# FederatedAI/FATE-LLM

Measured on AMD Instinct MI355X. Metric: GB/s param buffer reconstructed from (seed,scalar) list, device-resident, higher is better.
Workload: dtype bf16

## Files before the change

fate-llm_amd/csrc/fks_dev_update.h:

```cpp
#pragma once
#include <hip/hip_runtime.h>
#include <hip/hip_bf16.h>

#include "fks_internal.h"
#include "fks_dev_lds.h"

namespace fks {
namespace {

typedef __bf16 bf16x2_t __attribute__((ext_vector_type(2)));
__device__ __forceinline__ float rbf_cvt(float x) {
  const f32x2_t v = {0.0f, x};
  return __builtin_bit_cast(float, __builtin_convertvector(v, bf16x2_t));
}
__device__ __forceinline__ float rbf(float x) { return rbf_cvt(x); }
__device__ __forceinline__ float rhf(float x) {
  asm volatile("" : "+v"(x));
  return static_cast<float>(static_cast<_Float16>(x));
}

template <int DT>
struct Traits;

typedef __attribute__((address_space(1))) float gf32;
typedef __attribute__((address_space(1))) uint16_t gu16;
typedef __attribute__((address_space(1))) _Float16 gf16;

typedef __attribute__((address_space(1))) uint32_t gu32;

typedef __attribute__((address_space(1))) uint64_t gu64;

template <>
struct Traits<FKS_F32> {
  typedef uint64_t Pair;
  __device__ static Pair load_pair(uint64_t a) { return *reinterpret_cast<const gu64*>(a); }
  __device__ static void store_pair(uint64_t a, Pair v) { *reinterpret_cast<gu64*>(a) = v; }
  __device__ static uint32_t lo(Pair v) { return (uint32_t)v; }
  __device__ static uint32_t hi(Pair v) { return (uint32_t)(v >> 32); }
  __device__ static Pair pack(uint32_t l, uint32_t h) { return (uint64_t)l | ((uint64_t)h << 32); }
  __device__ static uint32_t bits(float v) { return __float_as_uint(v); }
  __device__ static uint32_t load_raw(uint64_t p, int64_t i) { return reinterpret_cast<const gu32*>(p)[i]; }
  __device__ static float cvt(uint32_t r) { return __uint_as_float(r); }
  __device__ static float load(uint64_t p, int64_t i) { return reinterpret_cast<const gf32*>(p)[i]; }
  __device__ static void store(uint64_t p, int64_t i, float v) { reinterpret_cast<gf32*>(p)[i] = v; }
  __device__ static float rnd(float x) { return x; }
};

template <>
struct Traits<FKS_BF16> {
  typedef uint32_t Pair;
  __device__ static Pair load_pair(uint64_t a) { return *reinterpret_cast<const gu32*>(a); }
  __device__ static void store_pair(uint64_t a, Pair v) { *reinterpret_cast<gu32*>(a) = v; }
  __device__ static uint32_t lo(Pair v) { return v & 0xffffu; }
  __device__ static uint32_t hi(Pair v) { return v >> 16; }
  __device__ static Pair pack(uint32_t l, uint32_t h) { return (l & 0xffffu) | (h << 16); }
  __device__ static uint32_t bits(float v) { return __float_as_uint(v) >> 16; }
  __device__ static uint32_t load_raw(uint64_t p, int64_t i) { return reinterpret_cast<const gu16*>(p)[i]; }
  __device__ static float cvt(uint32_t r) { return __uint_as_float(r << 16); }
  __device__ static float load(uint64_t p, int64_t i) {
    return __uint_as_float((uint32_t)reinterpret_cast<const gu16*>(p)[i] << 16);
  }
  __device__ static void store(uint64_t p, int64_t i, float v) {
    reinterpret_cast<gu16*>(p)[i] = (uint16_t)(__float_as_uint(v) >> 16);
  }
  __device__ static float rnd(float x) { return rbf(x); }
};

template <>
struct Traits<FKS_F16> {
  typedef uint32_t Pair;
  __device__ static Pair load_pair(uint64_t a) { return *reinterpret_cast<const gu32*>(a); }
  __device__ static void store_pair(uint64_t a, Pair v) { *reinterpret_cast<gu32*>(a) = v; }
  __device__ static uint32_t lo(Pair v) { return v & 0xffffu; }
  __device__ static uint32_t hi(Pair v) { return v >> 16; }
  __device__ static Pair pack(uint32_t l, uint32_t h) { return (l & 0xffffu) | (h << 16); }
  __device__ static uint32_t bits(float v) { return __builtin_bit_cast(uint16_t, static_cast<_Float16>(v)); }
  __device__ static uint32_t load_raw(uint64_t p, int64_t i) { return reinterpret_cast<const gu16*>(p)[i]; }
  __device__ static float cvt(uint32_t r) { return static_cast<float>(__builtin_bit_cast(_Float16, (uint16_t)r)); }
  __device__ static float load(uint64_t p, int64_t i) { return static_cast<float>(reinterpret_cast<const gf16*>(p)[i]); }
  __device__ static void store(uint64_t p, int64_t i, float v) { reinterpret_cast<gf16*>(p)[i] = static_cast<_Float16>(v); }
  __device__ static float rnd(float x) { return rhf(x); }
};

template <>
struct Traits<kDtF32Libm> : Traits<FKS_F32> {};
constexpr bool is_f32(int dt) { return dt == FKS_F32 || dt == kDtF32Libm; }

template <int DT>
__device__ __forceinline__ float apply_one(float p, float z, float g, float lr, float wd, bool has_wd, int mode,
                                           float ps, bool upd = true) {
  using TR = Traits<DT>;
  if (mode == kModeDelta) return __fmaf_rn(g, z, p);
  if (mode == kModePerturb || mode == kModePerturbUpdate) {
    p = TR::rnd(p + TR::rnd(ps * z));
    if (mode == kModePerturb || !upd) return p;
  }
  if (mode == kModeUpdate || mode == kModePerturbUpdate) {
    const float gz = TR::rnd(g * z);
    const float t2 = TR::rnd(gz + TR::rnd(wd * p));
    const float t = has_wd ? t2 : gz;
    return TR::rnd(p - TR::rnd(lr * t));
  }
  return z;
}

template <int DT>
__device__ __forceinline__ float dev_value_g(const float* v) {
  const float g = __int_as_float(__builtin_amdgcn_readfirstlane(__float_as_int(v[0])));
  return is_f32(DT) ? g : Traits<DT>::rnd(g);
}
__device__ __forceinline__ bool dev_value_apply(const float* v) {
  return __int_as_float(__builtin_amdgcn_readfirstlane(__float_as_int(v[1]))) != 0.0f;
}

template <int DT>
__device__ __forceinline__ f32x2_t rnd2(f32x2_t x) {
  f32x2_t r;
  r.x = Traits<DT>::rnd(x.x);
  r.y = Traits<DT>::rnd(x.y);
  return r;
}

template <int DT, int MODE>
__device__ __forceinline__ f32x2_t apply_tail(f32x2_t p, f32x2_t gz, float lr, float wd, bool has_wd) {
  f32x2_t t;
  if (MODE == kModeUpdateNoWd || MODE == kModeUpdateWdPos0) {
    t = gz;
  } else if (MODE == kModeUpdateWd0) {
    const f32x2_t ww = {wd, wd};
    t = __builtin_elementwise_fma(ww, p, gz);
  } else {
    const f32x2_t t2 = rnd2<DT>(gz + rnd2<DT>(wd * p));
    if (MODE == kModeUpdateWd) {
      t = t2;
    } else {
      t.x = has_wd ? t2.x : gz.x;
      t.y = has_wd ? t2.y : gz.y;
    }
  }
  return rnd2<DT>(p - rnd2<DT>(lr * t));
}

template <int DT, int MODE>
__device__ __forceinline__ f32x2_t apply_pair(f32x2_t p, f32x2_t z, float g, float lr, float wd, bool has_wd,
                                              float ps, bool upd = true) {
  if (MODE == kModeDelta) {
    const f32x2_t gg = {g, g};
    return __builtin_elementwise_fma(gg, z, p);
  }
  if (MODE == kModePerturb || MODE == kModePerturbUpdate) {
    p = rnd2<DT>(p + rnd2<DT>(ps * z));
    if (MODE == kModePerturb || !upd) return p;
  }
  if (MODE == kModeUpdate || MODE == kModeUpdateWd || MODE == kModeUpdateNoWd || MODE == kModePerturbUpdate ||
      MODE == kModeUpdateWd0 || MODE == kModeUpdateWdPos0)
    return apply_tail<DT, MODE>(p, rnd2<DT>(g * z), lr, wd, has_wd);
  return z;
}

__device__ __forceinline__ float mul_f16_ref(float a, float b, bool once) {
  if (once) {
    uint32_t r = 0;
    asm volatile("v_fma_mixlo_f16 %0, %1, %2, 0" : "+v"(r) : "v"(a), "v"(b));
    return (float)__builtin_bit_cast(_Float16, (uint16_t)(r & 0xffffu));
  }
  return rhf(a * b);
}
template <int MODE>
__device__ __forceinline__ f32x2_t apply_pair_f16dev(f32x2_t p, f32x2_t z, float g, float lr, float wd, bool has_wd,
                                                     float ps, bool upd, const bool (&once)[2],
                                                     const bool (&wd_once)[2]) {
  float q[2] = {p.x, p.y};
  const float zz[2] = {z.x, z.y};
  const bool use_wd = MODE == kModeUpdateNoWd ? false
                      : (MODE == kModeUpdateWd || MODE == kModeUpdateWd0 || MODE == kModeUpdateWdPos0) ? true
                                                                                                          : has_wd;
#pragma unroll
  for (int i = 0; i < 2; i++) {
    if (MODE == kModePerturb || MODE == kModePerturbUpdate) {
      q[i] = rhf(q[i] + mul_f16_ref(ps, zz[i], once[i]));
      if (MODE == kModePerturb || !upd) continue;
    }
    const float gz = mul_f16_ref(g, zz[i], once[i]);
    const float t = use_wd ? rhf(gz + mul_f16_ref(wd, q[i], wd_once[i])) : gz;
    q[i] = rhf(q[i] - mul_f16_ref(lr, t, once[i]));
  }
  return (f32x2_t){q[0], q[1]};
}

}
}
```

fate-llm_amd/csrc/fks_device.hip:

```cpp
#include <hip/hip_runtime.h>
#include <hip/hip_bf16.h>

#include <atomic>
#include <type_traits>
#include <mutex>

#include "fks_internal.h"
#include "fks_bitslice.h"
#define FKS_HD __device__ __forceinline__
#include "fks_libm.h"

constexpr int kDbMinWaves = 4;
constexpr int kZrUnroll = 2;
constexpr int kSm2MinWaves = 8;
constexpr int kBsFence = 8;
#ifndef FKS_BS_LAG
#define FKS_BS_LAG 36
#endif
#ifndef FKS_BS_R_VMEM
#define FKS_BS_R_VMEM 3
#endif
#ifndef FKS_PHX_VEC_ITEMS
#define FKS_PHX_VEC_ITEMS 8
#endif
#ifndef FKS_BS_WGTIME
#define FKS_BS_WGTIME 0
#endif

#include "fks_dev_lds.h"
#include "fks_dev_update.h"
#include "fks_dev_mt.h"
#include "fks_dev_zgen.h"
#include "fks_kern_jump.h"
#include "fks_kern_apply.h"
#include "fks_kern_slice.h"
#include "fks_kern_irregular.h"
#include "fks_kern_philox.h"
#include "fks_kern_selfcheck.h"

namespace fks {

int launch_delta_apply(const DeltaApplyDesc* d, int n, int64_t max_numel, const float* delta, void* stream) {
  const int64_t blocks = std::min<int64_t>(std::max<int64_t>(1, (max_numel + 255) / 256), 2048);
  hipLaunchKernelGGL(fks_delta_apply_kernel, dim3((unsigned)blocks, (unsigned)n), dim3(256), 0, (hipStream_t)stream,
                     d, delta);
  return (int)hipGetLastError();
}

static size_t apply_lds_bytes() { return (size_t)kLdsTabBytes + (size_t)kLdsStBytes; }

int device_cu_count() {
  int dev = 0, n = 0;
  if (hipGetDevice(&dev) != hipSuccess) return 256;
  if (hipDeviceGetAttribute(&n, hipDeviceAttributeMultiprocessorCount, dev) != hipSuccess || n <= 0) return 256;
  return n;
}

class PerDevice {
 public:
  template <class F>
  int run(F&& f) {
    int dev = 0;
    if (hipGetDevice(&dev) != hipSuccess || dev < 0 || dev >= 64) return -FKS_EINVAL;
    const uint64_t bit = 1ull << dev;
    if (done_.load(std::memory_order_acquire) & bit) return 0;
    std::lock_guard<std::mutex> lk(mu_);
    if (done_.load(std::memory_order_relaxed) & bit) return 0;
    const int e = f();
    if (e == 0) done_.fetch_or(bit, std::memory_order_release);
    return e;
  }

 private:
  std::mutex mu_;
  std::atomic<uint64_t> done_{0};
};

static int ensure_tables() {
  static PerDevice once;
  return once.run([] {
    const Tables& t = tables();
    static float buf[3 * 2048];
    for (int i = 0; i < 256; i++) {
      buf[i] = t.r_bf16[i];
      buf[256 + i] = t.c_bf16[i];
      buf[512 + i] = t.s_bf16[i];
    }
    hipError_t e = hipMemcpyToSymbol(HIP_SYMBOL(c_tab_bf16), buf, sizeof(float) * 768, 0, hipMemcpyHostToDevice);
    if (e != hipSuccess) return (int)e;
    for (int i = 0; i < 2048; i++) {
      buf[i] = t.r_f16[i];
      buf[2048 + i] = t.c_f16[i];
      buf[4096 + i] = t.s_f16[i];
    }
    e = hipMemcpyToSymbol(HIP_SYMBOL(c_tab_f16), buf, sizeof(buf), 0, hipMemcpyHostToDevice);
    return (int)e;
  });
}

template <class K>
static int ensure_lds_attr(PerDevice& once, K* fn, int bytes) {
  return once.run([&] {
    return (int)hipFuncSetAttribute(reinterpret_cast<const void*>(fn), hipFuncAttributeMaxDynamicSharedMemorySize,
                                    bytes);
  });
}

template <int... Vs>
struct IntList {};
template <int... Vs, class F>
static int dispatch(IntList<Vs...>, int v, F&& f) {
  int r = -FKS_ENOTSUP;
  (void)((v == Vs && (r = f(std::integral_constant<int, Vs>{}), true)) || ...);
  return r;
}

int launch_jump(const JumpArgs& a, int nseeds, void* stream) {
  const size_t lds = sizeof(uint32_t) * (size_t)kJumpLds2Words;
  static PerDevice attr;
  if (int e = ensure_lds_attr(attr, &fks_jump_kernel, (int)lds)) return e;
  dim3 grid((unsigned)nseeds, (unsigned)((a.nchunks + a.chunks_per_wg - 1) / a.chunks_per_wg));
  hipLaunchKernelGGL(fks_jump_kernel, grid, dim3(kJumpThreads), lds, (hipStream_t)stream, a);
  return (int)hipGetLastError();
}

template <int DT, int MODE, bool FULL, bool DB = false>
static int launch_apply_f(const ApplyArgs& a, void* stream) {
  const size_t lds = FULL ? apply_lds_bytes()
                          : (size_t)kLdsTabBytes + (size_t)((DB ? 2 : 1) * a.nseeds + 1) * kWinBytes;
  static PerDevice attr;
  if (int e = ensure_lds_attr(attr, &fks_apply_kernel<DT, MODE, FULL, DB>, (int)apply_lds_bytes())) return e;
  hipLaunchKernelGGL((fks_apply_kernel<DT, MODE, FULL, DB>), dim3((unsigned)a.nchunks),
                     dim3(DB ? kDbThreads : kApplyThreads), lds, (hipStream_t)stream, a);
  return (int)hipGetLastError();
}

template <int DT, int MODE, int ZM = 0>
static int launch_small2(const ApplyArgs& a, void* stream) {
  const size_t lds = (size_t)kLdsTabBytes + (size_t)(2 * a.nseeds + 1) * kWinBytes;
  static PerDevice attr;
  constexpr int kMaxLds = kLdsTabBytes + (2 * kSmallK + 1) * kWinBytes;
  if (int e = ensure_lds_attr(attr, &fks_small2_kernel<DT, MODE, ZM>, kMaxLds)) return e;
  hipLaunchKernelGGL((fks_small2_kernel<DT, MODE, ZM>), dim3((unsigned)a.nchunks), dim3(kSm2Threads), lds,
                     (hipStream_t)stream, a);
  return (int)hipGetLastError();
}

template <int DT, int MODE>
static int launch_apply_t(const ApplyArgs& a, void* stream) {
  if (a.nseeds == kMaxSeedsPerPass) return launch_apply_f<DT, MODE, true>(a, stream);
  if constexpr (DT == FKS_BF16) {
    if (a.zmode == 1 && a.nseeds == 1 && MODE == kModePerturb) return launch_small2<DT, MODE, 1>(a, stream);
    if (a.zmode == 2 && a.nseeds == 1 &&
        (MODE == kModePerturb || MODE == kModePerturbUpdate || MODE == kModeUpdate || MODE == kModeUpdateWd ||
         MODE == kModeUpdateNoWd || MODE == kModeUpdateWd0)) {
      hipLaunchKernelGGL((fks_zreplay_kernel<MODE>), dim3((unsigned)a.nchunks), dim3(kZrThreads), (size_t)3 * 1024,
                         (hipStream_t)stream, a);
      return (int)hipGetLastError();
    }
  }
  if (a.zmode == 2) return -FKS_ENOTSUP;
  if (a.nseeds <= kSmallK && DT != FKS_F16) return launch_small2<DT == FKS_F16 ? FKS_F32 : DT, MODE>(a, stream);
  if (a.nseeds <= kSmallK) return launch_apply_f<DT, MODE, false, true>(a, stream);
  return launch_apply_f<DT, MODE, false>(a, stream);
}

int launch_apply(int dtype, const ApplyArgs& a, void* stream) {
  if (a.nseeds < 1 || a.nseeds > kMaxSeedsPerPass || a.nchunks < 1) return -FKS_EINVAL;
  if (dtype == FKS_BF16) {
    int e = ensure_tables();
    if (e) return e;
  }
  using Modes = IntList<kModeUpdate, kModeUpdateWd, kModeUpdateNoWd, kModeUpdateWd0, kModePerturb, kModePerturbUpdate,
                        kModeWriteZ, kModeDelta>;
  return dispatch(IntList<FKS_F32, kDtF32Libm, FKS_BF16>{}, dtype, [&](auto dt) {
    return dispatch(Modes{}, a.mode,
                    [&](auto m) { return launch_apply_t<decltype(dt)::value, decltype(m)::value>(a, stream); });
  });
}

template <int MODE, bool FULL>
static int launch_apply_bs_m(const ApplyBsArgs& a, void* stream) {
  static PerDevice attr;
  if (int e = ensure_lds_attr(attr, &fks_apply_bs_kernel<MODE, FULL>, kBsLdsBytes)) return e;
  hipLaunchKernelGGL((fks_apply_bs_kernel<MODE, FULL>), dim3((unsigned)(a.split ? a.nchunks / 2 : a.nchunks)),
                     dim3(kBsThreads), kBsLdsBytes, (hipStream_t)stream, a);
  return (int)hipGetLastError();
}

template <int MODE>
static int launch_apply_bs_t(const ApplyBsArgs& a, void* stream) {
  const bool full = a.nseeds == (a.split ? kBsSeeds : kBsPassSeeds);
  return full ? launch_apply_bs_m<MODE, true>(a, stream) : launch_apply_bs_m<MODE, false>(a, stream);
}

int launch_apply_bs(const ApplyBsArgs& a, void* stream) {
  if (a.nseeds < 1 || a.nseeds > (a.split ? kBsSeeds : kBsPassSeeds) || a.nchunks < 1 ||
      (a.split && a.nchunks % 2))
    return -FKS_EINVAL;
  int e = ensure_tables();
  if (e) return e;
  return dispatch(IntList<kModeUpdate, kModeUpdateWd, kModeUpdateNoWd, kModeUpdateWd0, kModeDelta>{}, a.mode,
                  [&](auto m) { return launch_apply_bs_t<decltype(m)::value>(a, stream); });
}

template <int MODE>
static int launch_irregular_m(const IrrArgs& a, void* stream) {
  const size_t lds = (size_t)kIrrLogfOff + kLdsLogfBytes;
  static PerDevice attr;
  if (int e = ensure_lds_attr(attr, &fks_irregular_kernel<MODE>, (int)lds)) return e;
  hipLaunchKernelGGL((fks_irregular_kernel<MODE>), dim3((unsigned)a.nchunks), dim3(kApplyThreads), lds,
                     (hipStream_t)stream, a);
  return (int)hipGetLastError();
}

int launch_philox_fast_radius_check(uint32_t* counts, void* stream) {
  hipLaunchKernelGGL(fks_philox_fast_radius_kernel, dim3(kSqrtDomainBlocks), dim3(256), 0, (hipStream_t)stream, counts);
  return (int)hipGetLastError();
}

int launch_philox_radius_check(uint32_t* counts, void* stream) {
  hipLaunchKernelGGL(fks_philox_radius_kernel, dim3(kSqrtDomainBlocks), dim3(256), 0, (hipStream_t)stream, counts);
  return (int)hipGetLastError();
}

int launch_sqrt_domain_check(uint32_t* counts, void* stream) {
  hipLaunchKernelGGL(fks_sqrt_domain_kernel, dim3(kSqrtDomainBlocks), dim3(256), 0, (hipStream_t)stream, counts);
  return (int)hipGetLastError();
}

int device_max_threads_per_cu() {
  int dev = 0, n = 0;
  if (hipGetDevice(&dev) != hipSuccess) return 2048;
  if (hipDeviceGetAttribute(&n, hipDeviceAttributeMaxThreadsPerMultiProcessor, dev) != hipSuccess || n <= 0) return 2048;
  return n;
}

static int phx_vec_maxk() {
  static const int v = [] {
    const char* s = std::getenv("FKS_PHX_VEC_MAXK");
    return (s && *s) ? std::atoi(s) : kPhxSeeds;
  }();
  return v;
}

template <int MODE>
static int launch_philox_m(const PhiloxArgs& a, void* stream) {
  const int64_t items = a.item_hi - a.item_lo;
  if (items <= 0) return 0;
  if (a.nseeds <= phx_vec_maxk() && a.item_lo % kPhxVec == 0 && items % kPhxVec == 0) {
    const int64_t vitems = items / kPhxVec;
    const int64_t blocks = std::min<int64_t>((vitems + 255) / 256, (int64_t)device_cu_count() * 16);
    const size_t lds = a.nt <= kPhxLdsTensors ? sizeof(PhxTensor) * (size_t)a.nt : 0;
    hipLaunchKernelGGL((fks_philox_vec_kernel<MODE>), dim3((unsigned)blocks), dim3(256), lds, (hipStream_t)stream, a);
    return (int)hipGetLastError();
  }
  const int64_t blocks = std::min<int64_t>((items + 255) / 256, (int64_t)device_cu_count() * 16);
  hipLaunchKernelGGL((fks_philox_kernel<MODE>), dim3((unsigned)blocks), dim3(256), 0, (hipStream_t)stream, a);
  return (int)hipGetLastError();
}

int launch_philox(const PhiloxArgs& a, void* stream) {
  if (a.nseeds < 1 || a.nt < 1) return -FKS_EINVAL;
  using Modes = IntList<kModeUpdate, kModeUpdateWd, kModeUpdateNoWd, kModeUpdateWd0, kModeUpdateWdPos0, kModePerturb,
                        kModePerturbUpdate, kModeWriteZ, kModeDelta>;
  return dispatch(Modes{}, a.mode, [&](auto m) { return launch_philox_m<decltype(m)::value>(a, stream); });
}

int launch_irregular(const IrrArgs& a, void* stream) {
  if (a.nseeds < 1 || a.nseeds > kMaxSeedsPerPass) return -FKS_EINVAL;
  int e = ensure_tables();
  if (e) return e;
  return dispatch(IntList<kModeUpdate, kModePerturb, kModePerturbUpdate, kModeWriteZ, kModeDelta>{}, a.mode,
                  [&](auto m) { return launch_irregular_m<decltype(m)::value>(a, stream); });
}

}
```

fate-llm_amd/csrc/fks_kern_slice.h:

```cpp
#pragma once
#include <hip/hip_runtime.h>

#include "fks_internal.h"
#include "fks_bitslice.h"
#include "fks_dev_lds.h"
#include "fks_dev_update.h"
#include "fks_dev_zgen.h"

namespace fks {
namespace {

constexpr int kBsChunkBytes = kMtN * 16;
constexpr int kBsStateBytes = 8 * kBsChunkBytes;
constexpr int kBsTabBytes = 256 * 4 + 256 * 8;
constexpr uint32_t kBsFlagOff = kBsTabBytes + 2 * kBsStateBytes;
constexpr uint32_t kBsProgOff = kBsFlagOff + 8;
constexpr uint32_t kBsProg1Off = kBsProgOff + 4 * 6;
constexpr int kBsLdsBytes = (int)kBsProg1Off + 4 * 6;
static_assert(kBsLdsBytes <= 163840, "slice kernel LDS");
constexpr int kBsWaves = kBsHalfThreads / 64;
constexpr int kBsTaskWords = 128;

__device__ __forceinline__ void bs_store_row(uint32_t ra, const uint32_t (&x)[32]) {
#pragma unroll
  for (int q = 0; q < 8; q++) {
    const u32x4_t v = {x[4 * q], x[4 * q + 1], x[4 * q + 2], x[4 * q + 3]};
    lds_st4(ra + q * kBsChunkBytes, v);
  }
}

__device__ __forceinline__ uint32_t bs_flag_load(uint32_t off) {
  return *(volatile const lds_u32_t*)(size_t)off;
}
__device__ __forceinline__ void bs_flag_store(uint32_t off, uint32_t v) {
  asm volatile("" ::: "memory");
  __builtin_amdgcn_s_waitcnt(0xC07F);
  *(volatile lds_u32_t*)(size_t)off = v;
}

template <int S>
__device__ __forceinline__ uint32_t bs_index(uint32_t w, int c) {
  switch (c) {
    case 0: return bs::byte_x<0, S>(w);
    case 1: return bs::byte_x<1, S>(w);
    case 2: return bs::byte_x<2, S>(w);
    default: return bs::byte_x<3, S>(w);
  }
}

#if FKS_BS_WGTIME
__device__ uint64_t g_bs_wgtime[4096][16];
extern "C" int fks_debug_bs_wgtime(uint64_t* out, int nblocks) {
  return (int)hipMemcpyFromSymbol(out, HIP_SYMBOL(g_bs_wgtime), sizeof(uint64_t) * 16 * (size_t)nblocks, 0,
                                  hipMemcpyDeviceToHost);
}
#endif

template <int MODE, bool FULL>
__global__ __launch_bounds__(kBsThreads, 1) void fks_apply_bs_kernel(ApplyBsArgs a) {
  extern __shared__ __attribute__((aligned(16))) uint32_t lds32[];
  if ((uint32_t)(size_t)(lds_u32_t*)lds32 != 0u) __builtin_trap();
  const int tid = threadIdx.x;
  const int lane = tid & 63;
#if FKS_BS_WGTIME
  if (tid == 0) g_bs_wgtime[blockIdx.x][0] = __builtin_amdgcn_s_memrealtime();
  auto stamp = [&]() { if (lane == 0) g_bs_wgtime[blockIdx.x][1 + (tid >> 6)] = __builtin_amdgcn_s_memrealtime(); };
#else
  auto stamp = [&]() {};
#endif
  const int half = __builtin_amdgcn_readfirstlane(tid >= kBsHalfThreads ? 1 : 0);
  const int ht = tid - half * kBsHalfThreads;
  const int hw = __builtin_amdgcn_readfirstlane(ht >> 6);
  const bool split = a.split != 0;
  const int c = split ? 2 * (int)blockIdx.x + half : (int)blockIdx.x;
  const int nA = FULL ? kBsSeeds : split ? a.nseeds : (a.nseeds + 1) / 2;
  const int nseeds = FULL ? kBsSeeds : (half && !split ? a.nseeds - nA : nA);
  const int sfirst = half && !split ? nA : 0;
  const int64_t b0 = a.chunk_block[split ? c : 2 * c], b1 = a.chunk_block[split ? c + 1 : 2 * c + 2];
  const int nwords = (int)(kMtN * (b1 - b0));
  const int ntask = (nwords + kBsTaskWords - 1) / kBsTaskWords;
  const uint32_t sbase = kBsTabBytes + (uint32_t)half * kBsStateBytes;
  const uint32_t flag = kBsFlagOff + 4u * (uint32_t)half;

  for (int i = tid; i < 256; i += kBsThreads) {
    reinterpret_cast<float*>((uint8_t*)lds32)[i] = c_tab_bf16[i];
    reinterpret_cast<float2*>((uint8_t*)lds32 + 1024)[i] = make_float2(c_tab_bf16[256 + i], c_tab_bf16[512 + i]);
  }
  for (int i = ht; i < kMtN; i += kBsHalfThreads) {
    uint32_t w[32];
#pragma unroll
    for (int k = 0; k < 32; k++)
      w[k] = k < nseeds ? a.states[((size_t)(a.use_slot ? a.slot[sfirst + k] : (uint32_t)(sfirst + k)) * a.nchunks + c) *
                                       kMtN + i]
                        : 0u;
    bs::transpose32(w);
    bs_store_row(sbase + 16u * (uint32_t)i, w);
  }
  if (ht == 0) lds32[flag / 4] = 0u;
  if (ht < kBsWaves) lds32[(half ? kBsProg1Off : kBsProgOff) / 4 + ht] = 0u;
  __syncthreads();
  if (nseeds == 0) return;

  const int toff = 16 * (lane >> 3) + (lane & 7);
  const bool flip = ((lane >> 3) & 1) != 0;
  const bool odd = (lane & 1) != 0;

  float gk[kBsSeeds];
#pragma unroll
  for (int k = 0; k < kBsSeeds; k++) gk[k] = a.g[half ? k + sfirst : k];

  const int64_t wbase = (int64_t)kMtN * b0;
  int cur;
  {
    const int64_t s1 = wbase + (int64_t)kBsTaskWords * hw + toff;
    int lo = 0, hi = a.nsegs;
    while (lo < hi) {
      const int mid = (lo + hi) >> 1;
      if (a.segs[mid].start + a.segs[mid].numel <= s1) lo = mid + 1; else hi = mid;
    }
    cur = lo;
  }
  int64_t seg_start = INT64_MAX, seg_end = INT64_MAX;
  uint64_t seg_ptr = 0;
  float seg_lr = 0.0f, seg_wd = 0.0f;
  bool seg_wdf = false;
  constexpr int kEs = MODE == kModeDelta ? 4 : 2;
  constexpr bool kInc = MODE == kModeUpdateWd0;
  int seg_lo = INT32_MAX, seg_hi = INT32_MAX;
  uint64_t seg_org = 0;
  auto load_seg = [&]() {
    if (cur < a.nsegs) {
      const DevSeg sg = a.segs[cur];
      seg_start = sg.start;
      seg_end = sg.start + sg.numel;
      seg_ptr = sg.ptr;
      seg_lr = sg.lr;
      seg_wd = sg.wd;
      seg_wdf = (sg.flags & FKS_HAS_WD) != 0;
    } else {
      seg_start = seg_end = INT64_MAX;
    }
    if (kInc) {
      const int64_t lo = seg_start - wbase, hi = seg_end - wbase;
      seg_lo = (int)(lo < INT32_MIN ? INT32_MIN : lo > INT32_MAX ? INT32_MAX : lo);
      seg_hi = (int)(hi < INT32_MIN ? INT32_MIN : hi > INT32_MAX ? INT32_MAX : hi);
      seg_org = seg_ptr - (uint64_t)lo * kEs;
    }
    __builtin_amdgcn_s_waitcnt(0x0F70);
  };
  load_seg();

  using ST = Traits<MODE == kModeDelta ? FKS_F32 : FKS_BF16>;
  typedef typename ST::Pair Pair;
  struct Slot { uint64_t addr; float lr, wd; uint32_t wdf; Pair raw; };
  auto fetch = [&](int n) -> Slot {
    Slot sl;
    const int u1 = kBsTaskWords * n + toff;
    if (kInc) {
      while (u1 >= seg_hi) { cur++; load_seg(); }
      const bool on = u1 < nwords && u1 >= seg_lo;
      sl.lr = seg_lr; sl.wd = seg_wd; sl.wdf = seg_wdf;
      sl.addr = on ? seg_org + (uint64_t)(uint32_t)(u1 + (odd ? 7 : 0)) * kEs : (uint64_t)(uintptr_t)a.sink;
    } else {
      const int64_t s1 = wbase + u1;
      while (s1 >= seg_end) { cur++; load_seg(); }
      const bool on = u1 < nwords && s1 >= seg_start;
      sl.lr = seg_lr; sl.wd = seg_wd; sl.wdf = seg_wdf;
      sl.addr = on ? seg_ptr + (uint64_t)(s1 - seg_start + (odd ? 7 : 0)) * kEs : (uint64_t)(uintptr_t)a.sink;
    }
    sl.raw = ST::load_pair(sl.addr);
    return sl;
  };

  constexpr int kRowStep = kBsWaves * kBsTaskWords % kMtN;
  int row = (kBsTaskWords * hw + toff) % kMtN;
  auto next_row = [&]() {
    if (!kInc) return;
    row += kRowStep;
    if (row >= kMtN) row -= kMtN;
  };
  auto twist = [&](const int n, uint32_t (&oa)[8], uint32_t (&ob)[8]) {
    const int u1 = kBsTaskWords * n + toff;
    const bool valid = u1 < nwords;
    const int i1 = valid ? (kInc ? row : u1 % kMtN) : 0;
    const int ia = flip ? i1 + 8 : i1, ib = flip ? i1 : i1 + 8;
    auto rows = [&](int i, uint32_t& av, uint32_t& am, uint32_t& au) {
      const int iv = i + 1 < kMtN ? i + 1 : 0;
      const int im = i < kMtN - kMtM ? i + kMtM : i - (kMtN - kMtM);
      av = sbase + 16u * (uint32_t)iv;
      am = sbase + 16u * (uint32_t)im;
      au = sbase + 7u * kBsChunkBytes + 16u * (uint32_t)i + 12u;
    };
    uint32_t av1, am1, au1, av2, am2, au2;
    rows(ia, av1, am1, au1);
    rows(ib, av2, am2, au2);
    uint32_t M1[32], M2[32];
    const uint32_t U1 = lds_u32((int)au1), U2 = lds_u32((int)au2);
    u32x4_t va = lds_u4(av1), vb = lds_u4(av2), ma = lds_u4(am1), mb = lds_u4(am2);
    const uint32_t v0a = va.x, v0b = vb.x;
#pragma unroll
    for (int q = 0; q < 8; q++) {
      u32x4_t va2 = va, vb2 = vb, ma2 = ma, mb2 = mb;
      if (q < 7) {
        va2 = lds_u4(av1 + (q + 1) * kBsChunkBytes);
        vb2 = lds_u4(av2 + (q + 1) * kBsChunkBytes);
        ma2 = lds_u4(am1 + (q + 1) * kBsChunkBytes);
        mb2 = lds_u4(am2 + (q + 1) * kBsChunkBytes);
      }
      const uint32_t Va[5] = {va.x, va.y, va.z, va.w, va2.x};
      const uint32_t Vb[5] = {vb.x, vb.y, vb.z, vb.w, vb2.x};
      const uint32_t Ma[4] = {ma.x, ma.y, ma.z, ma.w}, Mb[4] = {mb.x, mb.y, mb.z, mb.w};
#pragma unroll
      for (int t = 0; t < 4; t++) {
        const int b = 4 * q + t;
        const bool am = ((bs::kMatrixA >> b) & 1u) != 0;
        uint32_t xa, xb;
        if (b < 30) { xa = Va[t + 1]; xb = Vb[t + 1]; }
        else if (b == 30) { xa = U1; xb = U2; }
        else { xa = 0u; xb = 0u; }
        M1[b] = am ? bs::xor3(Ma[t], xa, v0a) : (Ma[t] ^ xa);
        M2[b] = am ? bs::xor3(Mb[t], xb, v0b) : (Mb[t] ^ xb);
      }
      if (valid) {
        lds_st4(sbase + 16u * (uint32_t)ia + q * kBsChunkBytes, u32x4_t{M1[4 * q], M1[4 * q + 1], M1[4 * q + 2], M1[4 * q + 3]});
        lds_st4(sbase + 16u * (uint32_t)ib + q * kBsChunkBytes, u32x4_t{M2[4 * q], M2[4 * q + 1], M2[4 * q + 2], M2[4 * q + 3]});
      }
      va = va2; vb = vb2; ma = ma2; mb = mb2;
    }
    uint32_t o1[8], o2[8];
    bs::temper_low8(M1, o1);
    bs::temper_low8(M2, o2);
#pragma unroll
    for (int j = 0; j < 8; j++) {
      oa[j] = flip ? o2[j] : o1[j];
      ob[j] = flip ? o1[j] : o2[j];
    }
  };

  constexpr int kRv = kInc ? FKS_BS_R_VMEM : 0;
  static_assert(kRv >= 0 && kRv <= 8, "FKS_BS_R_VMEM");
  auto rv_slot = [](const int k) __attribute__((always_inline)) -> int {
    return (k & 7) < kRv ? (k >> 3) * kRv + (k & 7) : -1;
  };
  auto chain_head = [&](uint32_t (&oa)[8], uint32_t (&ob)[8], float (&rv)[4 * kRv + 1]) {
    bs::transpose8(oa);
    bs::transpose8(ob);
#pragma unroll
    for (int k = 0; k < kBsSeeds; k++)
      if (rv_slot(k) >= 0)
        rv[rv_slot(k)] =
            *reinterpret_cast<const float*>(reinterpret_cast<const char*>(c_tab_bf16) + bs_index<2>(oa[k & 7], k >> 3));
  };
  auto chain = [&](const Slot& sl, uint32_t (&oa)[8], uint32_t (&ob)[8], const float (&rv)[4 * kRv + 1]) {
    if (kRv == 0) {
      bs::transpose8(oa);
      bs::transpose8(ob);
    }
    f32x2_t p;
    {
      const uint32_t keep = odd ? ST::hi(sl.raw) : ST::lo(sl.raw);
      const uint32_t got = swap_adjacent(odd ? ST::lo(sl.raw) : ST::hi(sl.raw));
      p.x = ST::cvt(odd ? got : keep);
      p.y = ST::cvt(odd ? keep : got);
    }
    auto z_of = [&](const int k) __attribute__((always_inline)) -> f32x2_t {
      const float r = rv_slot(k) >= 0 ? rv[rv_slot(k)] : lds_f32(bs_index<2>(oa[k & 7], k >> 3));
      const f32x2_t rr = {r, r}, zero = {0.0f, 0.0f};
      const f32x2_t cs = lds_f32x2(1024u + bs_index<3>(ob[k & 7], k >> 3));
      return rnd2<FKS_BF16>(__builtin_elementwise_fma(rr, cs, zero));
    };
    {
#pragma unroll
      for (int k = 0; k < kBsSeeds; k++) {
        if (FULL || k < nseeds) p = apply_pair<FKS_BF16, MODE>(p, z_of(k), gk[k], sl.lr, sl.wd, sl.wdf != 0, 0.0f);
        if ((k % kBsFence) == kBsFence - 1) asm volatile("" ::: "memory");
      }
    }
    const uint32_t b1v = ST::bits(p.x), b2v = ST::bits(p.y);
    const uint32_t back = swap_adjacent(odd ? b1v : b2v);
    const Pair out = odd ? ST::pack(back, b2v) : ST::pack(b1v, back);
    ST::store_pair(sl.addr, out);
  };

  const bool ordered = !split;
  const uint32_t prog = kBsProgOff + 4u * (uint32_t)hw;
  auto publish_stored = [&](const int m) {
    asm volatile("" ::: "memory");
    __builtin_amdgcn_s_waitcnt(0x0F70);
    if (lane == 0) *(volatile lds_u32_t*)(size_t)prog = (uint32_t)m + 1u;
  };
  auto await_stored = [&](const int m) {
    if (m >= ntask) return;
    const uint32_t pm = kBsProgOff + 4u * (uint32_t)(m % kBsWaves);
    while (__builtin_amdgcn_readfirstlane(bs_flag_load(pm)) < (uint32_t)m + 1u) __builtin_amdgcn_s_sleep(1);
    asm volatile("" ::: "memory");
  };
  static_assert(FKS_BS_LAG == 0 || FKS_BS_LAG > 2 * kBsWaves, "FKS_BS_LAG: half 1 trails by 12 tasks");
  constexpr bool kLag = FKS_BS_LAG > 0 && (MODE == kModeUpdateWd || MODE == kModeUpdate);
  const uint32_t prog1 = kBsProg1Off + 4u * (uint32_t)hw;
  auto publish_applied = [&](const int m) {
    if (lane == 0) *(volatile lds_u32_t*)(size_t)prog1 = (uint32_t)m + 1u;
  };
  auto await_applied = [&](const int m) {
    if (m < 0) return;
    const uint32_t pm = kBsProg1Off + 4u * (uint32_t)(m % kBsWaves);
    while (__builtin_amdgcn_readfirstlane(bs_flag_load(pm)) < (uint32_t)m + 1u) __builtin_amdgcn_s_sleep(1);
  };

  auto task = [&](const int n, const Slot& sl, Slot& nx) {
    uint32_t oa[8], ob[8];
    if (kLag && ordered && half == 0) await_applied(n - FKS_BS_LAG);
    __builtin_amdgcn_s_setprio(2);
    while (__builtin_amdgcn_readfirstlane(bs_flag_load(flag)) < (uint32_t)n) __builtin_amdgcn_s_sleep(0);
    asm volatile("" ::: "memory");
    twist(n, oa, ob);
    if (lane == 0) bs_flag_store(flag, (uint32_t)n + 1u);
    __builtin_amdgcn_s_setprio(0);
    if (ordered && half == 0) {
      if (n >= kBsWaves) publish_stored(n - kBsWaves);
    } else if (ordered) {
      await_stored(n + kBsWaves);
    }
    float rv[4 * kRv + 1];
    if (kRv > 0) chain_head(oa, ob, rv);
    nx = fetch(n + kBsWaves);
    chain(sl, oa, ob, rv);
    if (kLag && ordered && half) publish_applied(n);
  };

  if (hw >= ntask) { stamp(); return; }
  if (ordered && half) await_stored(hw);
  Slot s0 = fetch(hw), s1;
  int n = hw;
  for (;;) {
    task(n, s0, s1);
    if (n + kBsWaves >= ntask) break;
    n += kBsWaves;
    next_row();
    task(n, s1, s0);
    if (n + kBsWaves >= ntask) break;
    n += kBsWaves;
    next_row();
  }
  if (ordered && half == 0) publish_stored(n);
  stamp();
}

}
}
```

Baseline: 1.273.

## Use d16-hi bf16 loads/stores, SGPR-packed seed scalars, and branchless row/flip muxing

For the weight-decay-zero update mode, each lane now loads and stores its two bf16 parameters directly as high-half 16-bit accesses 16 bytes apart. This replaces the 32-bit pair load plus cross-lane swap_adjacent shuffle. Per-seed scalars are packed into 64-bit uniform pairs so the g*z multiply can use v_pk_mul_f32 with an SGPR operand. Row wrapping and flip selection become branchless min/mux forms to cut VALU and select instructions. In exchange, memory access changes from one 32-bit transaction to two 16-bit ones per lane, and the code relies on inline asm op_sel semantics.

```diff
diff --git a/fate-llm_amd/csrc/fks_dev_update.h b/fate-llm_amd/csrc/fks_dev_update.h
--- a/fate-llm_amd/csrc/fks_dev_update.h
+++ b/fate-llm_amd/csrc/fks_dev_update.h
@@ -29,6 +29,7 @@
 typedef __attribute__((address_space(1))) uint32_t gu32;
 
 typedef __attribute__((address_space(1))) uint64_t gu64;
+typedef uint16_t u16x2_t __attribute__((ext_vector_type(2)));
 
 template <>
 struct Traits<FKS_F32> {
@@ -54,6 +55,11 @@
   __device__ static uint32_t lo(Pair v) { return v & 0xffffu; }
   __device__ static uint32_t hi(Pair v) { return v >> 16; }
   __device__ static Pair pack(uint32_t l, uint32_t h) { return (l & 0xffffu) | (h << 16); }
+  __device__ static uint32_t load_hi(uint64_t a) {
+    const u16x2_t v = {(uint16_t)0, *reinterpret_cast<const gu16*>(a)};
+    return __builtin_bit_cast(uint32_t, v);
+  }
+  __device__ static void store_hi(uint64_t a, uint32_t v) { *reinterpret_cast<gu16*>(a) = (uint16_t)(v >> 16); }
   __device__ static uint32_t bits(float v) { return __float_as_uint(v) >> 16; }
   __device__ static uint32_t load_raw(uint64_t p, int64_t i) { return reinterpret_cast<const gu16*>(p)[i]; }
   __device__ static float cvt(uint32_t r) { return __uint_as_float(r << 16); }
@@ -118,6 +124,16 @@
   f32x2_t r;
   r.x = Traits<DT>::rnd(x.x);
   r.y = Traits<DT>::rnd(x.y);
+  return r;
+}
+
+template <int H>
+__device__ __forceinline__ f32x2_t pk_mul_half(uint64_t gg, f32x2_t z) {
+  f32x2_t r;
+  if (H == 0)
+    asm("v_pk_mul_f32 %0, %1, %2 op_sel:[0,0] op_sel_hi:[0,1]" : "=v"(r) : "s"(gg), "v"(z));
+  else
+    asm("v_pk_mul_f32 %0, %1, %2 op_sel:[1,0] op_sel_hi:[1,1]" : "=v"(r) : "s"(gg), "v"(z));
   return r;
 }
 
diff --git a/fate-llm_amd/csrc/fks_device.hip b/fate-llm_amd/csrc/fks_device.hip
--- a/fate-llm_amd/csrc/fks_device.hip
+++ b/fate-llm_amd/csrc/fks_device.hip
@@ -19,6 +19,18 @@
 #endif
 #ifndef FKS_BS_R_VMEM
 #define FKS_BS_R_VMEM 3
+#endif
+#ifndef FKS_BS_D16
+#define FKS_BS_D16 1
+#endif
+#ifndef FKS_BS_G32
+#define FKS_BS_G32 1
+#endif
+#ifndef FKS_BS_ROWMIN
+#define FKS_BS_ROWMIN 1
+#endif
+#ifndef FKS_BS_FLIPMUX
+#define FKS_BS_FLIPMUX 1
 #endif
 #ifndef FKS_PHX_VEC_ITEMS
 #define FKS_PHX_VEC_ITEMS 8
diff --git a/fate-llm_amd/csrc/fks_kern_slice.h b/fate-llm_amd/csrc/fks_kern_slice.h
--- a/fate-llm_amd/csrc/fks_kern_slice.h
+++ b/fate-llm_amd/csrc/fks_kern_slice.h
@@ -105,9 +105,21 @@
   const bool flip = ((lane >> 3) & 1) != 0;
   const bool odd = (lane & 1) != 0;
 
+  constexpr bool kWd0 = MODE == kModeUpdateWd0;
+  constexpr bool kD16 = kWd0 && FKS_BS_D16 != 0;
+  constexpr bool kG32 = kWd0 && FKS_BS_G32 != 0;
+  constexpr bool kRowMin = kWd0 && FKS_BS_ROWMIN != 0;
+  constexpr bool kFlipMux = kWd0 && FKS_BS_FLIPMUX != 0;
+  uint32_t flipm = flip ? ~0u : 0u;
+  if (kFlipMux) asm volatile("" : "+v"(flipm));
+
   float gk[kBsSeeds];
 #pragma unroll
   for (int k = 0; k < kBsSeeds; k++) gk[k] = a.g[half ? k + sfirst : k];
+  uint64_t gg[kBsSeeds / 2];
+#pragma unroll
+  for (int k = 0; k < kBsSeeds / 2; k++)
+    gg[k] = (uint64_t)rfl(__float_as_uint(gk[2 * k])) | ((uint64_t)rfl(__float_as_uint(gk[2 * k + 1])) << 32);
 
   const int64_t wbase = (int64_t)kMtN * b0;
   int cur;
@@ -152,7 +164,7 @@
 
   using ST = Traits<MODE == kModeDelta ? FKS_F32 : FKS_BF16>;
   typedef typename ST::Pair Pair;
-  struct Slot { uint64_t addr; float lr, wd; uint32_t wdf; Pair raw; };
+  struct Slot { uint64_t addr; float lr, wd; uint32_t wdf; Pair raw; uint32_t hi0, hi1; };
   auto fetch = [&](int n) -> Slot {
     Slot sl;
     const int u1 = kBsTaskWords * n + toff;
@@ -160,7 +172,12 @@
       while (u1 >= seg_hi) { cur++; load_seg(); }
       const bool on = u1 < nwords && u1 >= seg_lo;
       sl.lr = seg_lr; sl.wd = seg_wd; sl.wdf = seg_wdf;
-      sl.addr = on ? seg_org + (uint64_t)(uint32_t)(u1 + (odd ? 7 : 0)) * kEs : (uint64_t)(uintptr_t)a.sink;
+      sl.addr = on ? seg_org + (uint64_t)(uint32_t)(u1 + (odd && !kD16 ? 7 : 0)) * kEs : (uint64_t)(uintptr_t)a.sink;
+      if (kD16) {
+        sl.hi0 = Traits<FKS_BF16>::load_hi(sl.addr);
+        sl.hi1 = Traits<FKS_BF16>::load_hi(sl.addr + 16);
+        return sl;
+      }
     } else {
       const int64_t s1 = wbase + u1;
       while (s1 >= seg_end) { cur++; load_seg(); }
@@ -174,19 +191,29 @@
 
   constexpr int kRowStep = kBsWaves * kBsTaskWords % kMtN;
   int row = (kBsTaskWords * hw + toff) % kMtN;
+  auto wrap = [](uint32_t x) -> uint32_t {
+    const uint32_t y = x - (uint32_t)kMtN;
+    return x < y ? x : y;
+  };
+  uint32_t rofa = flip ? 8u : 0u, rofb = flip ? 0u : 8u;
+  if (kRowMin) asm volatile("" : "+v"(rofa), "+v"(rofb));
   auto next_row = [&]() {
     if (!kInc) return;
+    if (kRowMin) {
+      row = (int)wrap((uint32_t)row + kRowStep);
+      return;
+    }
     row += kRowStep;
     if (row >= kMtN) row -= kMtN;
   };
   auto twist = [&](const int n, uint32_t (&oa)[8], uint32_t (&ob)[8]) {
     const int u1 = kBsTaskWords * n + toff;
     const bool valid = u1 < nwords;
-    const int i1 = valid ? (kInc ? row : u1 % kMtN) : 0;
-    const int ia = flip ? i1 + 8 : i1, ib = flip ? i1 : i1 + 8;
+    const int i1 = kRowMin ? row : valid ? (kInc ? row : u1 % kMtN) : 0;
+    const int ia = kRowMin ? i1 + (int)rofa : flip ? i1 + 8 : i1, ib = kRowMin ? i1 + (int)rofb : flip ? i1 : i1 + 8;
     auto rows = [&](int i, uint32_t& av, uint32_t& am, uint32_t& au) {
-      const int iv = i + 1 < kMtN ? i + 1 : 0;
-      const int im = i < kMtN - kMtM ? i + kMtM : i - (kMtN - kMtM);
+      const int iv = kRowMin ? (int)wrap((uint32_t)i + 1u) : i + 1 < kMtN ? i + 1 : 0;
+      const int im = kRowMin ? (int)wrap((uint32_t)i + kMtM) : i < kMtN - kMtM ? i + kMtM : i - (kMtN - kMtM);
       av = sbase + 16u * (uint32_t)iv;
       am = sbase + 16u * (uint32_t)im;
       au = sbase + 7u * kBsChunkBytes + 16u * (uint32_t)i + 12u;
@@ -232,8 +259,8 @@
     bs::temper_low8(M2, o2);
 #pragma unroll
     for (int j = 0; j < 8; j++) {
-      oa[j] = flip ? o2[j] : o1[j];
-      ob[j] = flip ? o1[j] : o2[j];
+      oa[j] = kFlipMux ? bs::mux(flipm, o2[j], o1[j]) : flip ? o2[j] : o1[j];
+      ob[j] = kFlipMux ? bs::mux(flipm, o1[j], o2[j]) : flip ? o1[j] : o2[j];
     }
   };
 
@@ -257,7 +284,10 @@
       bs::transpose8(ob);
     }
     f32x2_t p;
-    {
+    if (kD16) {
+      p.x = __uint_as_float(sl.hi0);
+      p.y = __uint_as_float(sl.hi1);
+    } else {
       const uint32_t keep = odd ? ST::hi(sl.raw) : ST::lo(sl.raw);
       const uint32_t got = swap_adjacent(odd ? ST::lo(sl.raw) : ST::hi(sl.raw));
       p.x = ST::cvt(odd ? got : keep);
@@ -272,9 +302,20 @@
     {
 #pragma unroll
       for (int k = 0; k < kBsSeeds; k++) {
-        if (FULL || k < nseeds) p = apply_pair<FKS_BF16, MODE>(p, z_of(k), gk[k], sl.lr, sl.wd, sl.wdf != 0, 0.0f);
+        if (FULL || k < nseeds) {
+          if (kG32)
+            p = apply_tail<FKS_BF16, MODE>(p, rnd2<FKS_BF16>(k & 1 ? pk_mul_half<1>(gg[k >> 1], z_of(k)) : pk_mul_half<0>(gg[k >> 1], z_of(k))),
+                                           sl.lr, sl.wd, sl.wdf != 0);
+          else
+            p = apply_pair<FKS_BF16, MODE>(p, z_of(k), gk[k], sl.lr, sl.wd, sl.wdf != 0, 0.0f);
+        }
         if ((k % kBsFence) == kBsFence - 1) asm volatile("" ::: "memory");
       }
+    }
+    if (kD16) {
+      Traits<FKS_BF16>::store_hi(sl.addr, __float_as_uint(p.x));
+      Traits<FKS_BF16>::store_hi(sl.addr + 16, __float_as_uint(p.y));
+      return;
     }
     const uint32_t b1v = ST::bits(p.x), b2v = ST::bits(p.y);
     const uint32_t back = swap_adjacent(odd ? b1v : b2v);
```

Result: faster. 1.290 (median of 6 runs) (+1.4%).
